# Liupeter01/Software-Rasterizer

Hardware: AMD Instinct MI355X
Metric: frames_per_sec (higher is better)
Workload: dtype f32

## Files before the change

software-rasterizer_amd/csrc/srz_api.hip:

```cpp
#include <dlfcn.h>

#include <algorithm>
#include <cmath>
#include <cstdio>
#include <cstdlib>
#include <cstring>
#include <initializer_list>
#include <new>
#include <string>
#include <vector>

#include "srz_device.h"

using namespace srz;

namespace {
std::string g_create_error;

struct EventPair {
  hipEvent_t t0, t1, t2, t3;
  bool detailed;
};

struct BatchDesc {
// ... 12 lines not shown

struct srz_ctx {
  int device = 0;
  hipStream_t stream = nullptr;
  std::string err;
  int shard_rank = 0, shard_world = 1;
  TexDesc h_tex[MAX_TEX];
  uint32_t *d_texmem[MAX_TEX];
  unsigned long long *d_stats = nullptr;
  struct MeshSlot {
    srz_vertex *d_verts = nullptr;
    uint32_t *d_faces = nullptr;
    uint32_t *d_corner_off = nullptr;
    uint32_t n_verts = 0, n_faces = 0;
    uint64_t upload = 0;
  } mesh[MAX_MESH];
  uint64_t mesh_uploads = 0;
  int timing = 0;
  std::vector<EventPair> ev_pool, ev_used;
  double acc_ms[4] = {0, 0, 0, 0};
  uint64_t tex_version = 1;
  int acc_launches = 0;
  std::vector<float> acc_samples;
  hipEvent_t span_t0 = nullptr;
  bool span_open = false;
  double span_ms = 0.0;
  unsigned long long dbg[ST_COUNT] = {};
  srz_frameset *draw_fs = nullptr;
  float *draw_out = nullptr;
  std::vector<uint64_t> draw_sig;
  int env_sub_batch = 0;
  bool env_no_packed = false;
  uint32_t env_clear_wgs = 0;
  std::vector<std::pair<uint64_t, uint32_t>> clear_memo;
  bool opt_approx_shade = false;
  bool opt_pool_lazy = false;
  static constexpr int EV_RING = 8;
  hipStream_t stream2 = nullptr;
  hipEvent_t ev_fork[EV_RING] = {}, ev_join[EV_RING] = {};
  float *batch_out = nullptr;
  size_t batch_out_bytes = 0;
  hipStream_t stream3 = nullptr;
  hipEvent_t ev_piece[EV_RING] = {};
  unsigned ev_next = 0;
  hipEvent_t ev_raster[EV_RING] = {};
  unsigned raster_next = 0;
  hipStream_t raster_last_stream = nullptr;
  bool raster_valid = false;
};

struct srz_target {
  int width = 0, height = 0;
  float *d_planes = nullptr;
  uint8_t *d_bgr8 = nullptr;
// ... 53 lines not shown
  std::vector<uint64_t> h_draw_upload;
  uint32_t n_draws = 0, max_faces = 0;
  uint64_t sdesc_version = 0;
  uint32_t tiles_x = 0, max_tiles = 0;
  bool have_stats = false;
  bool update_failed = false;
  static constexpr int CLEAR_TUNE_SKIP = 6, CLEAR_TUNE_AGAIN = 4096;
  struct ClearTune {
    uint32_t wgs = CLEAR_GRID_DEFAULT;
    bool done = false;
    int renders = 0;
    int since = 0;
    ClearCtl *d_ctl = nullptr;
    uint32_t *h_wgs = nullptr;
  } clear_tune;
  srz_stats stats{};
};

namespace {

hipStream_t pick_stream(const srz_ctx *ctx, void *stream) {
  if (!stream) return ctx->stream;
  return stream == SRZ_STREAM_NULL ? (hipStream_t) nullptr : (hipStream_t)stream;
}

int fail(srz_ctx *ctx, int code, const std::string &msg) {
  if (ctx)
    ctx->err = msg;
  else
    g_create_error = msg;
// ... 69 lines not shown
  for (int i = 0; i < srz_frameset::STAGE_RING; ++i) {
    if (fs->h_stage[i]) (void)hipHostFree(fs->h_stage[i]);
    if (fs->stage_ev[i]) (void)hipEventDestroy(fs->stage_ev[i]);
  }
  (void)hipFree(fs->d_dyn);
  (void)hipFree(fs->d_tris);
  (void)hipFree(fs->d_tri_pos);
  (void)hipFree(fs->d_bbox);
  (void)hipFree(fs->d_tri_batch);
  (void)hipFree(fs->d_pool);
  (void)hipFree(fs->d_pool_heads);
  if (fs->h_pool_heads) (void)hipHostFree(fs->h_pool_heads);
  if (fs->clear_tune.h_wgs) (void)hipHostFree(fs->clear_tune.h_wgs), fs->clear_tune.h_wgs = nullptr;
  if (fs->clear_tune.d_ctl) (void)hipFree(fs->clear_tune.d_ctl), fs->clear_tune.d_ctl = nullptr;
  (void)hipFree(fs->d_tile_info);
  (void)hipFree(fs->d_sparse_rows);
  (void)hipFree(fs->d_slow_list);
  (void)hipFree(fs->d_slow_count);
  (void)hipFree(fs->d_redo_list);
  (void)hipFree(fs->d_vis);
  (void)hipFree(fs->d_worklist);
  (void)hipFree(fs->d_work_count);
  (void)hipFree(fs->d_chunk_rows);
  (void)hipFree(fs->d_band_desc);
  (void)hipFree(fs->d_band_ent);
  (void)hipFree(fs->d_sdesc);
}

struct Pass {
  enum Kind { COLOUR, VISIBILITY, COUNTING, SIZE_ONLY, PEEL } kind = COLOUR;
// ... 217 lines not shown
  return SRZ_OK;
}

void end_clear_plan(srz_frameset *fs, const ClearPlan &p, hipStream_t s) {
  if (p.count) ++fs->clear_tune.renders;
  if (p.stamp) launch_clear_tune(fs->clear_tune.d_ctl, fs->clear_tune.h_wgs, s);
  if (p.rebase) launch_clear_rebase(fs->clear_tune.d_ctl, s);
}

struct RenderPlan {
  Pass pass;
  hipStream_t s;
  bool side, turns, vertex_setup;
  ClearPlan clear;
  EventPair *ep;
};

int enqueue_sub_batch(srz_ctx *ctx, srz_frameset *fs, const RenderPlan &r, RenderArgs &a, int f0, int n, int part) {
  const bool stats = r.pass.kind == Pass::COUNTING;
  const hipStream_t s = r.s;
  const size_t tpf = (size_t)fs->n_local_bands * fs->tiles_x;
  RenderArgs v = a;
  if (n != fs->n_frames) {
    const int fa = r.pass.f_begin + f0;
    v.frames += fa, v.n_frames = (uint32_t)n;
    v.vis += (size_t)fa * tpf * ((size_t)TILE * TILE);
    v.tile_info += (size_t)fa * tpf;
    v.out += (size_t)fa * a.frame_stride;
    v.work_cap = (uint32_t)((size_t)(n < 8 ? n : (n + 7) / 8) * tpf);
  }
  const uint32_t tiles = (uint32_t)((size_t)n * tpf);
  if (r.vertex_setup) launch_chunks(v, n, fs->max_tris, s);
  else launch_setup(v, n, fs->max_tris, stats, s);
  launch_bin(v, n, fs->max_tris, s);
  if (!fs->pool_sized && !stats) {
    HIP_TRY(ctx, copy_demand(fs, part, s));
    HIP_TRY(ctx, hipStreamSynchronize(s));
    const uint32_t need = max_pool_demand(fs, part, part + 1);
    if (need > fs->pool_sub_cap) {
      if (int rc = grow_pool(ctx, fs, need, 8u)) return rc;
      a.pool = v.pool = fs->d_pool, a.pool_sub_cap = v.pool_sub_cap = fs->pool_sub_cap;
      HIP_TRY(ctx, hipMemsetAsync(fs->d_pool_heads, 0, sizeof(uint32_t) * CNT_STRIDE * fs->pool_n_sub, s));
      launch_bin(v, n, fs->max_tris, s);
    }
  }
  if (r.pass.kind == Pass::SIZE_ONLY) return SRZ_OK;
  if (r.ep) HIP_TRY(ctx, hipEventRecord(r.ep->t1, s));
  const unsigned ev = r.side ? ctx->ev_next++ % srz_ctx::EV_RING : 0u;
  if (r.side) {
    HIP_TRY(ctx, hipEventRecord(ctx->ev_fork[ev], s));
    HIP_TRY(ctx, hipStreamWaitEvent(ctx->stream2, ctx->ev_fork[ev], 0));
    launch_clear(v, tiles, ctx->stream2, r.clear.wgs);
    HIP_TRY(ctx, copy_demand(fs, part, ctx->stream2));
    HIP_TRY(ctx, hipEventRecord(ctx->ev_join[ev], ctx->stream2));
  }
  if (r.pass.kind == Pass::PEEL) launch_peel(v, r.pass.d_prev + (v.out - a.out), n, s);
  else launch_raster(v, n, stats, s);
  if (r.turns) {
    HIP_TRY(ctx, hipEventRecord(ctx->ev_raster[ctx->raster_next++ % srz_ctx::EV_RING], s));
    ctx->raster_last_stream = s, ctx->raster_valid = true;
  }
  if (r.ep) HIP_TRY(ctx, hipEventRecord(r.ep->t2, s));
  if (r.pass.writes_visibility()) launch_visibility(v, tiles, s);
  else launch_shade(v, tiles, stats, fs->fast_kinds, fs->any_generic, fs->approx_shade, s);
  if (r.side) HIP_TRY(ctx, hipStreamWaitEvent(s, ctx->ev_join[ev], 0));
  else if (r.pass.kind == Pass::PEEL || !raster_four_waves(v))
    HIP_TRY(ctx, copy_demand(fs, part, s));
// ... 23 lines not shown
    if (int rc = begin_timing(ctx, ep, detailed, s)) return rc;
  if (stats) HIP_TRY(ctx, hipMemsetAsync(ctx->d_stats, 0, ST_COUNT * sizeof(unsigned long long), s));
  if (fs->max_tris == 0) {
    HIP_TRY(ctx, hipMemsetAsync(fs->d_work_count, 0, sizeof(uint32_t) * CNT_STRIDE * N_WORK_LISTS, s));
    HIP_TRY(ctx, hipMemsetAsync(fs->d_pool_heads, 0, sizeof(uint32_t) * CNT_STRIDE * fs->pool_n_sub, s));
    HIP_TRY(ctx, hipMemsetAsync(fs->d_slow_count, 0, 2 * sizeof(uint32_t), s));
  }
  const bool turns = !stats && !size_only && fs->max_tiles >= 8192;
  if (turns && !ctx->ev_raster[0])
    if (int rc = create_side(ctx, "render: raster events", nullptr, false, ctx->ev_raster)) return rc;
  if (turns && ctx->raster_valid && ctx->raster_last_stream != s) {
    HIP_TRY(ctx, hipStreamWaitEvent(s, ctx->ev_raster[(ctx->raster_next + srz_ctx::EV_RING - 1) % srz_ctx::EV_RING], 0));
    a.other_streams = 1u;
  }
  const bool vertex_setup = fs->d_draws != nullptr && !stats;
  if (fs->d_draws) launch_vertex(fs->d_draws, fs->n_draws, fs->max_faces, fs->d_tris, fs->d_tri_pos, fs->d_frames, vertex_setup ? fs->d_bbox : nullptr, s);
  const bool any_fused = any_frame_has(fs, flags_or, SRZ_FUSED_CLEAR), side = any_fused && fs->max_tiles >= 8192 && !size_only;
  if (side && !ctx->stream2)
    if (int rc = create_side(ctx, "render: clear stream", &ctx->stream2, true, ctx->ev_fork, ctx->ev_join)) return rc;
  if (!side && any_fused) a.clear_in_raster = 1u;
  RenderPlan r{pass, s, side, turns, vertex_setup, ClearPlan{}, detailed ? &ep : nullptr};
  if (side)
    if (int rc = plan_clear(ctx, fs, pass, detailed, s, r.clear)) return rc;
  a.clear_wgs_dev = r.clear.dev_wgs;
  const int n_all = pass.f_count < 0 ? fs->n_frames : pass.f_count;
  const int chunk = sub_batch_frames(ctx, fs, n_all, stats || detailed);
  for (int f0 = 0, part = 0; f0 < n_all; f0 += chunk, ++part)
    if (int rc = enqueue_sub_batch(ctx, fs, r, a, f0, std::min(chunk, n_all - f0), part)) return rc;
  if (!stats) fs->pool_sized = true;
  end_clear_plan(fs, r.clear, s);
  if (timed) {
    HIP_TRY(ctx, hipEventRecord(ep.t3, s));
    ctx->ev_used.push_back(ep);
  }
  HIP_TRY(ctx, hipGetLastError());
  return SRZ_OK;
}

int render_entry(const char *name, srz_ctx *ctx, srz_frameset *fs, void *d_out, size_t out_bytes, uint32_t flags, void *stream, Pass pass) {
  if (!ctx) return SRZ_E_INVALID;
  const std::string fn(name);
  if (!fs || !d_out) return fail(ctx, SRZ_E_INVALID, fn + ": null frameset / output");
  if (out_bytes < srz_frameset_out_bytes(ctx, fs)) return fail(ctx, SRZ_E_INVALID, fn + ": output buffer too small");
  if (((uintptr_t)d_out & 15u) != 0) return fail(ctx, SRZ_E_INVALID, fn + ": output must be 16-byte aligned");
// ... 322 lines not shown

void srz_destroy(srz_ctx *ctx) {
  if (!ctx) return;
  (void)hipSetDevice(ctx->device);
  (void)hipStreamSynchronize(ctx->stream);
  if (ctx->draw_fs) srz_frameset_destroy(ctx, ctx->draw_fs);
  (void)hipFree(ctx->draw_out);
  (void)hipFree(ctx->batch_out);
  if (ctx->span_t0) (void)hipEventDestroy(ctx->span_t0);
  for (auto &ep : ctx->ev_used) ctx->ev_pool.push_back(ep);
  for (auto &ep : ctx->ev_pool) (void)hipEventDestroy(ep.t0), (void)hipEventDestroy(ep.t1), (void)hipEventDestroy(ep.t2), (void)hipEventDestroy(ep.t3);
  for (int i = 0; i < MAX_TEX; ++i) (void)hipFree(ctx->d_texmem[i]);
  for (int i = 0; i < MAX_MESH; ++i) (void)hipFree(ctx->mesh[i].d_verts), (void)hipFree(ctx->mesh[i].d_faces), (void)hipFree(ctx->mesh[i].d_corner_off);
  (void)hipFree(ctx->d_stats);
  destroy_side(ctx->stream2, ctx->ev_fork, ctx->ev_join);
  destroy_side(ctx->stream3, ctx->ev_piece);
  destroy_side(nullptr, ctx->ev_raster);
  (void)hipStreamDestroy(ctx->stream);
  delete ctx;
}

const char *srz_last_error(const srz_ctx *ctx) { return ctx ? ctx->err.c_str() : g_create_error.c_str(); }

int srz_set_option(srz_ctx *ctx, int option, int value) {
  if (!ctx) return SRZ_E_INVALID;
  if (option == SRZ_OPT_POOL_LAZY)
    ctx->opt_pool_lazy = value != 0;
  else if (option == SRZ_OPT_APPROX_SHADE)
    ctx->opt_approx_shade = value != 0;
  else
// ... 187 lines not shown
    const uint64_t n_wgs = (uint64_t)((n_frames + 7) / 8 * 8) * fs->n_local_bands;
    uint32_t n_sub = 1;
    while (n_sub < 64u && (uint64_t)n_sub * 256u <= n_wgs) n_sub *= 2u;
    fs->pool_n_sub = n_sub;
    const uint64_t cap = std::min<uint64_t>((4ull * tri_off + 4096u) / n_sub + 64u, 0xfffffff0ull / n_sub);
    fs->pool_sub_cap = (uint32_t)cap;
    FS_TRY(dev_alloc((void **)&fs->d_pool, sizeof(uint32_t) * cap * n_sub));
    FS_TRY(dev_alloc((void **)&fs->d_pool_heads, sizeof(uint32_t) * CNT_STRIDE * 64));
    FS_TRY(hipHostMalloc((void **)&fs->h_pool_heads, sizeof(uint32_t) * CNT_STRIDE * 64 * srz_frameset::DEMAND_PARTS, hipHostMallocMapped | hipHostMallocCoherent));
    if (e == hipSuccess) std::memset(fs->h_pool_heads, 0, sizeof(uint32_t) * CNT_STRIDE * 64 * srz_frameset::DEMAND_PARTS);
    FS_TRY(dev_alloc((void **)&fs->clear_tune.d_ctl, sizeof(ClearCtl)));
    if (e == hipSuccess) FS_TRY(hipMemset(fs->clear_tune.d_ctl, 0, sizeof(ClearCtl)));
    FS_TRY(hipHostMalloc((void **)&fs->clear_tune.h_wgs, 64, hipHostMallocMapped | hipHostMallocCoherent));
    if (e == hipSuccess) *fs->clear_tune.h_wgs = 0u;
    FS_TRY(dev_alloc((void **)&fs->d_tile_info, sizeof(uint2) * fs->max_tiles));
    FS_TRY(dev_alloc((void **)&fs->d_slow_list, sizeof(uint32_t) * fs->max_tiles));
    FS_TRY(dev_alloc((void **)&fs->d_slow_count, 2 * sizeof(uint32_t)));
    FS_TRY(dev_alloc((void **)&fs->d_redo_list, sizeof(uint4) * fs->max_tiles));
  }
  FS_TRY(dev_alloc((void **)&fs->d_vis, sizeof(uint32_t) * (size_t)fs->max_tiles * ((size_t)TILE * TILE)));
  FS_TRY(ensure_worklists(fs));
  FS_TRY(dev_alloc((void **)&fs->d_work_count, sizeof(uint32_t) * CNT_STRIDE * N_WORK_LISTS));
  FS_TRY(dev_alloc((void **)&fs->d_sdesc, sizeof(ShadeDescG) * fs->h_batches.size()));
  std::vector<uint8_t> h_dyn(fs->dyn_bytes);
  stage_dyn(fs, h_dyn.data());
  FS_TRY(hipMemcpy(fs->d_dyn, h_dyn.data(), fs->dyn_bytes, hipMemcpyHostToDevice));
  if (tri_off) {
    if (copy_tris) FS_TRY(hipMemcpy(fs->d_tris, h_tris.data(), sizeof(srz_tri) * tri_off, hipMemcpyHostToDevice));
    if (!h_pos.empty()) FS_TRY(hipMemcpy(fs->d_tri_pos, h_pos.data(), sizeof(float) * h_pos.size(), hipMemcpyHostToDevice));
    FS_TRY(hipMemcpy(fs->d_tri_batch, h_tb.data(), sizeof(uint16_t) * tri_off, hipMemcpyHostToDevice));
// ... 39 lines not shown
  {
    std::vector<uint32_t> at(off, off + n_verts);
    for (uint32_t i = 0; i < 3u * n_faces; ++i) corners[at[faces[i]]++] = i;
  }
  srz_ctx::MeshSlot m;
  HIP_TRY(ctx, hipMalloc(&m.d_verts, sizeof(srz_vertex) * n_verts));
  hipError_t e = hipMalloc(&m.d_faces, sizeof(uint32_t) * 3 * (n_faces ? n_faces : 1));
  if (e == hipSuccess) e = hipMalloc(&m.d_corner_off, sizeof(uint32_t) * lists.size());
  if (e == hipSuccess) e = hipMemcpy(m.d_verts, verts, sizeof(srz_vertex) * n_verts, hipMemcpyHostToDevice);
  if (e == hipSuccess && n_faces) e = hipMemcpy(m.d_faces, faces, sizeof(uint32_t) * 3 * n_faces, hipMemcpyHostToDevice);
  if (e == hipSuccess) e = hipMemcpy(m.d_corner_off, lists.data(), sizeof(uint32_t) * lists.size(), hipMemcpyHostToDevice);
  if (e != hipSuccess) {
    (void)hipFree(m.d_verts), (void)hipFree(m.d_faces), (void)hipFree(m.d_corner_off);
    return fail(ctx, SRZ_E_NOMEM, std::string("srz_mesh_upload: ") + hipGetErrorString(e));
  }
  m.n_verts = n_verts, m.n_faces = n_faces, m.upload = ++ctx->mesh_uploads;
  (void)hipStreamSynchronize(ctx->stream);
  (void)hipFree(ctx->mesh[mesh_id].d_verts), (void)hipFree(ctx->mesh[mesh_id].d_faces), (void)hipFree(ctx->mesh[mesh_id].d_corner_off);
  ctx->mesh[mesh_id] = m;
  return SRZ_OK;
}

int srz_mesh_update(srz_ctx *ctx, int mesh_id, const srz_vertex *d_verts, uint32_t n_verts, void *stream) {
  if (!ctx) return SRZ_E_INVALID;
  const std::string fn("srz_mesh_update");
  if (mesh_id < 0 || mesh_id >= MAX_MESH || !ctx->mesh[mesh_id].d_verts) return fail(ctx, SRZ_E_INVALID, fn + ": no mesh in that slot");
  if (!d_verts) return fail(ctx, SRZ_E_INVALID, fn + ": null vertices");
  const srz_ctx::MeshSlot &m = ctx->mesh[mesh_id];
  if (n_verts != m.n_verts) return fail(ctx, SRZ_E_INVALID, fn + ": n_verts is not the slot's vertex count");
  if (!aligned<4>({d_verts})) return fail(ctx, SRZ_E_INVALID, fn + ": the vertices must be 4-byte aligned");
  HIP_TRY(ctx, hipSetDevice(ctx->device));
  HIP_TRY(ctx, hipMemcpyAsync(m.d_verts, d_verts, sizeof(srz_vertex) * n_verts, hipMemcpyDeviceToDevice, pick_stream(ctx, stream)));
  return SRZ_OK;
}

static int check_mesh_normals(srz_ctx *ctx, const std::string &fn, int mesh_id, const float *d_pos, uint32_t pos_stride, uint32_t n_sets,
                              MeshNormalsArgs &a, size_t *pos_span) {
  if (mesh_id < 0 || mesh_id >= MAX_MESH || !ctx->mesh[mesh_id].d_verts) return fail(ctx, SRZ_E_INVALID, fn + ": no mesh in that slot");
  const srz_ctx::MeshSlot &m = ctx->mesh[mesh_id];
  if (n_sets == 0u || n_sets > 65535u) return fail(ctx, SRZ_E_INVALID, fn + ": n_sets must be 1 .. 65535");
  if (!d_pos && n_sets != 1u) return fail(ctx, SRZ_E_INVALID, fn + ": the slot's own vertices are one set (n_sets must be 1)");
  if (d_pos && pos_stride < 3u) return fail(ctx, SRZ_E_INVALID, fn + ": pos_stride must be at least 3");
  a.pos = d_pos ? d_pos : reinterpret_cast<const float *>(m.d_verts), a.pos_stride = d_pos ? pos_stride : 8u;
  a.faces = m.d_faces, a.corner_off = m.d_corner_off, a.corners = m.d_corner_off + m.n_verts + 1;
  a.n_verts = m.n_verts, a.n_sets = n_sets;
  *pos_span = (((size_t)n_sets * m.n_verts - 1u) * a.pos_stride + 3u) * sizeof(float);
// ... 140 lines not shown
      const srz_ctx::MeshSlot &m = ctx->mesh[dr.mesh_id];
      DrawDesc dd{};
      dd.verts = m.d_verts, dd.faces = m.d_faces, dd.n_faces = m.n_faces, dd.tri_off = first, dd.frame = (uint32_t)f;
      set_draw(dd, sf, dr);
      draws.push_back(dd), draw_mesh.push_back(dr.mesh_id), draw_upload.push_back(m.upload);
      first += m.n_faces;
    }
  }
  std::vector<srz_frame> fr;
  std::vector<srz_batch> batches;
  scene_frames(ctx, frames, n_frames, fr, batches);
  srz_frameset *fs = nullptr;
  int rc = build_frameset(ctx, fr.data(), n_frames, &fs, false, false, &draws);
  if (rc) return rc;
  fs->h_draw_mesh = draw_mesh, fs->h_draw_upload = draw_upload;
  *out = fs;
  return size_pool ? size_pool_at_create(ctx, out) : SRZ_OK;
}

int srz_sceneset_update(srz_ctx *ctx, srz_frameset *fs, const srz_scene_frame *frames, int n_frames) {
  if (!ctx) return SRZ_E_INVALID;
  if (!fs || !frames || !fs->d_draws) return fail(ctx, SRZ_E_INVALID, "srz_sceneset_update: not a sceneset");
  if (n_frames != fs->n_frames) return fail(ctx, SRZ_E_INVALID, "srz_sceneset_update: frame count changed");
  HIP_TRY(ctx, hipSetDevice(ctx->device));
  for (int f = 0, di = 0; f < n_frames; ++f) {
    const srz_scene_frame &sf = frames[f];
    const FrameDesc &d = fs->h_frames[f];
    if (sf.width != fs->width || sf.height != fs->height || sf.n_lights != d.n_lights || sf.n_draws != d.n_batches ||
        (sf.n_lights && !sf.lights) || (sf.n_draws && !sf.draws))
      return fail(ctx, SRZ_E_INVALID, "srz_sceneset_update: structure changed");
    for (uint32_t k = 0; k < sf.n_draws; ++k, ++di) {
      const srz_mesh_draw &dr = sf.draws[k];
      if (dr.mesh_id != fs->h_draw_mesh[di] || dr.mesh_id < 0 || dr.mesh_id >= MAX_MESH ||
          ctx->mesh[dr.mesh_id].n_faces != fs->h_draws[di].n_faces || ctx->mesh[dr.mesh_id].upload != fs->h_draw_upload[di])
        return fail(ctx, SRZ_E_INVALID, "srz_sceneset_update: mesh binding changed");
    }
  }
  for (int f = 0, di = 0; f < n_frames; ++f)
    for (uint32_t k = 0; k < frames[f].n_draws; ++k) set_draw(fs->h_draws[di++], frames[f], frames[f].draws[k]);
  std::vector<srz_frame> fr;
  std::vector<srz_batch> batches;
  scene_frames(ctx, frames, n_frames, fr, batches);
  return refresh_frames(ctx, fs, fr.data(), n_frames, "srz_sceneset_update", false);
}

int srz_target_create(srz_ctx *ctx, int width, int height, srz_target **out) {
  if (!ctx) return SRZ_E_INVALID;
  if (!out || width <= 0 || height <= 0 || width > 32767 || height > 32767) return fail(ctx, SRZ_E_INVALID, "srz_target_create: bad size");
  *out = nullptr;
  HIP_TRY(ctx, hipSetDevice(ctx->device));
  srz_target *t = new (std::nothrow) srz_target();
  if (!t) return fail(ctx, SRZ_E_NOMEM, "srz_target_create: out of host memory");
  t->width = width, t->height = height;
  const size_t plane = (size_t)width * height;
// ... 1598 lines not shown
  unsigned long long h[5];
  HIP_TRY(ctx, hipMemcpyAsync(h, ctx->d_stats, sizeof h, hipMemcpyDeviceToHost, ctx->stream));
  HIP_TRY(ctx, hipStreamSynchronize(ctx->stream));
  for (int i = 0; i < 5; ++i) out5[i] = h[i];
  return SRZ_OK;
}

int srz_debug_counters(srz_ctx *ctx, uint64_t *out, int n) {
  if (!ctx || !out) return SRZ_E_INVALID;
#ifdef SRZ_PHASE_PROBE
  (void)hipDeviceSynchronize();
  (void)hipMemcpy(ctx->dbg, ctx->d_stats, sizeof ctx->dbg, hipMemcpyDeviceToHost);
  (void)hipMemset(ctx->d_stats, 0, sizeof ctx->dbg);
#endif
  for (int i = 0; i < n && i < ST_COUNT; ++i) out[i] = ctx->dbg[i];
  return ST_COUNT;
}

}
namespace {
struct RcclApi {
  void *handle = nullptr;
  struct UniqueId { char internal[128]; };
  int (*GetUniqueId)(UniqueId *) = nullptr;
  int (*CommInitRank)(void **, int, UniqueId, int) = nullptr;
  int (*AllGather)(const void *, void *, size_t, int, void *, hipStream_t) = nullptr;
  int (*CommDestroy)(void *) = nullptr;
  const char *(*GetErrorString)(int) = nullptr;
  std::string error;
};
RcclApi &rccl() {
// ... 305 lines not shown
  for (int f = 0; f < n_frames; ++f) {
    const srz_frame &fr = frames[f];
    const FrameDesc &d = fs->h_frames[f];
    if (fr.width != fs->width || fr.height != fs->height) return bad(SRZ_E_INVALID, "frame size changed");
    if (fr.n_lights != d.n_lights || (fr.n_lights && !fr.lights)) return bad(SRZ_E_INVALID, "light count changed");
    if (fr.n_batches != d.n_batches || (fr.n_batches && !fr.batches)) return bad(SRZ_E_INVALID, "batch count changed");
    for (uint32_t b = 0; b < fr.n_batches; ++b) {
      const srz_batch &sb = fr.batches[b];
      if (sb.n_tris != fs->h_batches[d.batch_off + b].count) return bad(SRZ_E_INVALID, "triangle count of a batch changed");
      if (sb.shader < SRZ_SHADER_NORMAL || sb.shader > SRZ_SHADER_BUMP) return bad(SRZ_E_INVALID, "unknown shader type");
      if (copy_tris && sb.n_tris && !sb.tris) return bad(SRZ_E_INVALID, "batch with null triangle pointer");
    }
  }
  if (int rc = ensure_stage_ring(ctx, fs, who)) return rc;
  bool batches_changed = false;
  for (int f = 0; f < n_frames; ++f) {
    const srz_frame &fr = frames[f];
    FrameDesc &d = fs->h_frames[f];
    set_shading(d, fr);
    if (fr.n_lights) std::memcpy(&fs->h_lights[d.light_off], fr.lights, sizeof(srz_light) * fr.n_lights);
    for (uint32_t b = 0; b < fr.n_batches; ++b) {
      BatchDesc &bd = fs->h_batches[d.batch_off + b];
      if (bd.shader != fr.batches[b].shader || bd.tex_id != fr.batches[b].tex_id)
        bd.shader = fr.batches[b].shader, bd.tex_id = fr.batches[b].tex_id, batches_changed = true;
    }
  }
  classify_frames(fs);
  fs->update_failed = ensure_worklists(fs) != hipSuccess;
  if (fs->update_failed) return bad(SRZ_E_NOMEM, "hipMalloc of the work lists failed");
  if (int rc = upload_dyn(ctx, fs)) return rc;
  if (batches_changed) fs->sdesc_version = 0;
  if (copy_tris) {
    for (int f = 0; f < n_frames; ++f) {
      size_t o = fs->h_frames[f].tri_off;
      for (uint32_t b = 0; b < frames[f].n_batches; ++b) {
        const srz_batch &sb = frames[f].batches[b];
        if (sb.n_tris) HIP_TRY(ctx, hipMemcpyAsync(fs->d_tris + o, sb.tris, sizeof(srz_tri) * sb.n_tris, hipMemcpyHostToDevice, ctx->stream));
        o += sb.n_tris;
      }
    }
  }
// ... 146 lines not shown
```

software-rasterizer_amd/csrc/srz_device.h:

```cpp
#pragma once
#include <hip/hip_runtime.h>
#include <stdint.h>

#include "../../include/srz.h"

namespace srz {

constexpr int TILE = 32;
constexpr int BAND = 32;
constexpr int KEY_STRIDE = TILE + 1;
constexpr int LDS_STRIDE = 32;
#ifndef SRZ_BAND_ROT
#define SRZ_BAND_ROT 5
#endif
__host__ __device__ inline int band_rot(int world) { return (SRZ_BAND_ROT % world) ? SRZ_BAND_ROT : (SRZ_BAND_ROT ? 1 : 0); }
__host__ __device__ inline int band_of(int lb, int rank, int world) {
  if (world == 1) return lb;
  int j = (rank - band_rot(world) * lb) % world;
  return lb * world + (j < 0 ? j + world : j);
}
__host__ __device__ inline int rank_of_band(int b, int world) { return (b + band_rot(world) * (b / world)) % world; }
constexpr uint32_t NO_TRI = 0xffffffffu;
constexpr uint32_t CNT_STRIDE = 32;
constexpr uint32_t FD_FAST_SHADE = 0x100u, FD_NL_SHIFT = 9;
// ... 89 lines not shown
  uint4 *redo_list;
  uint32_t *redo_count;
  uint32_t *vis;
  uint4 *worklist;
  uint64_t kind_slots;
  uint32_t *work_count;
  uint32_t work_cap;
  uint32_t tiles_x, n_local_bands, n_frames;
  float *out;
  uint64_t frame_stride;
  uint32_t local_rows;
  int32_t shard_rank, shard_world;
  uint32_t flags_or;
  unsigned long long *stats;
  const uint32_t *clear_wgs_dev;
};

constexpr int CLEAR_CANDS = 3, CLEAR_TUNE_BLOCK = 3, CLEAR_TUNE_RENDERS = 2 * CLEAR_CANDS * CLEAR_TUNE_BLOCK;
constexpr uint32_t CLEAR_CAND[CLEAR_CANDS] = {96, 128, 256};
constexpr uint32_t CLEAR_GRID_MAX = 256, CLEAR_GRID_DEFAULT = 96;
struct ClearCtl {
  uint32_t wgs;
  uint32_t cur, pos, phase, done, alive;
  uint32_t n[CLEAR_CANDS];
  unsigned long long last;
  float t[CLEAR_CANDS][4];
  float score[CLEAR_CANDS];
};
void launch_clear_tune(ClearCtl *ctl, uint32_t *h_wgs, hipStream_t s);
void launch_clear_rebase(ClearCtl *ctl, hipStream_t s);

// ... 50 lines not shown
  const float *attr;
  float *out;
  const float *gout;
  float *gattr;
  uint64_t attr_frame_stride;
  uint32_t n_verts, n_ch, pos_tris, n_frames;
};
void launch_corner_attr(const CornerAttrArgs &a, hipStream_t s);
void launch_corner_attr_grad(const CornerAttrArgs &a, hipStream_t s);
void launch_chunks(const RenderArgs &a, int n_frames, uint32_t max_tris, hipStream_t s);
void launch_setup(const RenderArgs &a, int n_frames, uint32_t max_tris, bool stats, hipStream_t s);
void launch_bin(const RenderArgs &a, int n_frames, uint32_t max_tris, hipStream_t s);
void launch_raster(const RenderArgs &a, int n_frames, bool stats, hipStream_t s);
void launch_peel(const RenderArgs &a, const float *prev, int n_frames, hipStream_t s);
bool raster_four_waves(const RenderArgs &a);
void launch_clear(const RenderArgs &a, uint32_t max_tiles, hipStream_t s, uint32_t wgs);
void launch_shade(const RenderArgs &a, uint32_t max_tiles, bool stats, uint32_t kinds, bool any_generic, bool approx, hipStream_t s);
void launch_visibility(const RenderArgs &a, uint32_t max_tiles, hipStream_t s);
struct ShadeVisArgs {
  const FrameDesc *frames;
  const srz_tri *tris;
  const uint16_t *tri_batch;
  const srz_light *lights;
  const ShadeDescG *sdesc;
  const float *vis;
  float *out;
  uint64_t frame_stride;
  uint32_t local_rows, tiles_x, n_local_bands, n_frames;
  int32_t shard_rank, shard_world;
  uint32_t flags_or, in_place;
  uint32_t any_generic;
// ... 439 lines not shown
```

software-rasterizer_amd/csrc/srz_kernels.hip:

```cpp
#include "srz_device.h"

#include <algorithm>
#include <cstdio>
#include <cstdlib>
#include <type_traits>

#pragma clang fp contract(off)

namespace srz {

#define SRZ_CAS __attribute__((address_space(4)))
template <typename T> __device__ __forceinline__ const SRZ_CAS T *as_const(const T *p) { return (const SRZ_CAS T *)(p); }
typedef float f32x4 __attribute__((ext_vector_type(4)));
typedef unsigned int u32x2 __attribute__((ext_vector_type(2)));
typedef unsigned int u32x4 __attribute__((ext_vector_type(4)));

__device__ __forceinline__ float sse_max(float a, float b) { return a > b ? a : b; }
__device__ __forceinline__ float sse_min(float a, float b) { return a < b ? a : b; }
__device__ __forceinline__ float std_max(float a, float b) { return (a < b) ? b : a; }
__device__ __forceinline__ float std_clamp(float v, float lo, float hi) { return (v < lo) ? lo : (hi < v) ? hi : v; }
__device__ __forceinline__ float fmsubf(float a, float b, float c) { return __builtin_fmaf(a, b, -c); }
__device__ __forceinline__ float fmaf_(float a, float b, float c) { return __builtin_fmaf(a, b, c); }

__device__ __forceinline__ uint32_t f2u_(float f) { return __builtin_bit_cast(uint32_t, f); }
// ... 2215 lines not shown
    float *gz = rc.out0 + (size_t)ly * W + x4;
    const bool full = vec_ok && x4 + 3 <= rc.tx1;
    if (tile_has_owner)
      quad_store(gz, rc.plane, {z4}, full, x4, rc.tx1);
    else
      quad_store(gz, rc.plane, {z4, zero4, zero4, zero4}, full, x4, rc.tx1);
  }
  if (tile_has_owner) {
    uint32_t *slot = a.vis + ((size_t)frame * tiles_per_frame + tile) * PIX_SLOT;
    for (int it = 0; it < 4; ++it) ids_store4(slot, (uint32_t)((it * 8 + (lane >> 3)) * TILE + (lane & 7) * 4), id4[it], false, false);
    if (lane == 0) work_append(a, fd->flags, frame * tiles_per_frame + tile, work_entry(frame, lb, tx, false, false, 0u, 0u));
  }
}

__global__ __launch_bounds__(256) void k_clear(RenderArgs a) {
  const uint32_t n_items = a.n_frames * a.n_local_bands * 4u;
  const float inf = __builtin_inff();
  uint32_t n_wgs = gridDim.x;
  if (a.clear_wgs_dev) {
    const uint32_t w = *as_const(a.clear_wgs_dev);
    n_wgs = min(w ? w : CLEAR_CAND[0], gridDim.x);
    if (blockIdx.x >= n_wgs) return;
  }
  for (uint32_t it = blockIdx.x; it < n_items; it += n_wgs) {
    const uint32_t br = it >> 2, pl = it & 3u;
    const uint32_t f = br / a.n_local_bands, lb = br % a.n_local_bands;
    const SRZ_CAS FrameDesc *fd = as_const(a.frames) + f;
    if (!((fd->flags | a.flags_or) & SRZ_FUSED_CLEAR)) continue;
    const int W = fd->width, H = fd->height;
    const int band = band_of((int)lb, a.shard_rank, a.shard_world);
    const int rows = min(BAND, H - band * BAND);
    const size_t plane = (size_t)a.local_rows * (size_t)W;
    float *base = a.out + (size_t)f * a.frame_stride + (size_t)lb * BAND * (size_t)W + pl * plane;
    const float v = pl == 0u ? inf : 0.f;
    const float4 v4 = make_float4(v, v, v, v);
    const SRZ_CAS u32x2 *cnt = as_const(reinterpret_cast<const u32x2 *>(a.tile_info)) + (size_t)br * a.tiles_x;
    for (int x4 = (int)threadIdx.x * 4; x4 < W; x4 += (int)blockDim.x * 4) {
      if (cnt[(uint32_t)x4 / TILE].x != 0u) continue;
      if (((W & 3) == 0)) {
        for (int ly = 0; ly < rows; ++ly) store_nt(base + (size_t)ly * W + x4, v4);
      } else {
        for (int ly = 0; ly < rows; ++ly)
          for (int k = 0; k < 4 && x4 + k < W; ++k) base[(size_t)ly * W + x4 + k] = v;
      }
    }
  }
}


#ifndef SRZ_FAST_MINW
#define SRZ_FAST_MINW 6
#endif
#ifndef SRZ_STAGE_TRIS
// ... 5332 lines not shown
  }
  int arg = -1;
  for (int i = 0; i < CLEAR_CANDS; ++i)
    if ((c->alive >> i & 1u) && (arg < 0 || c->score[i] < c->score[arg])) arg = i;
  c->wgs = CLEAR_CAND[arg < 0 ? 0 : arg], c->done = 1u;
  __hip_atomic_store(h_wgs, c->wgs, __ATOMIC_RELEASE, __HIP_MEMORY_SCOPE_SYSTEM);
}

void launch_clear_tune(ClearCtl *ctl, uint32_t *h_wgs, hipStream_t s) { hipLaunchKernelGGL(k_clear_tune, dim3(1), dim3(1), 0, s, ctl, h_wgs); }

__global__ void k_clear_rebase(ClearCtl *c) {
  if (!c->done) c->last = __builtin_amdgcn_s_memrealtime();
}
void launch_clear_rebase(ClearCtl *ctl, hipStream_t s) { hipLaunchKernelGGL(k_clear_rebase, dim3(1), dim3(1), 0, s, ctl); }

void launch_clear(const RenderArgs &a, uint32_t max_tiles, hipStream_t s, uint32_t wgs) {
  if (max_tiles == 0) return;
  const uint32_t n_items = a.n_frames * a.n_local_bands * 4u;
  const uint32_t cap = wgs ? wgs : 96u;
  hipLaunchKernelGGL(k_clear, dim3(n_items < cap ? n_items : cap), dim3(256), 0, s, a);
}

static uint32_t tile_grid(uint32_t items, uint32_t cap = 16384u) { return (std::min(items, cap) + 7u) & ~7u; }

static dim3 shade_grid(const RenderArgs &a, uint32_t max_tiles) { return dim3(tile_grid(max_tiles, a.other_streams ? 2048u : 16384u)); }

template <int FASTNL, bool BUMPY, class L> static void launch_kind(uint32_t kinds, bool approx, L &launch) {
  if (!((kinds >> build_kind<FASTNL, BUMPY>()) & 1u)) return;
  if constexpr (FASTNL > 0 && !BUMPY)
    if (approx) return launch(std::integral_constant<int, FASTNL>{}, std::false_type{}, std::true_type{});
  launch(std::integral_constant<int, FASTNL>{}, std::bool_constant<BUMPY>{}, std::false_type{});
}
template <class L> static void launch_fast_kinds(uint32_t kinds, bool approx, L &&launch) {
  launch_kind<1, false>(kinds, approx, launch), launch_kind<2, false>(kinds, approx, launch);
  launch_kind<3, false>(kinds, approx, launch), launch_kind<4, false>(kinds, approx, launch);
// ... 177 lines not shown
```

Before: 331,600.

## Start fused clear early using cached per-tile coverage mask across renders

Adds a per-frame, per-band bitmask of tiles that have triangles. It is rebuilt only when geometry, the eye position or the meshes change. When the mask is valid, the first slice of the clear kernel is launched on the side stream before vertex setup and binning, and the rest after binning, so clearing overlaps geometry work instead of waiting behind it. Vertex launch is moved into the sub-batch path. The risk is a stale mask if a geometry change is missed, which would produce wrong output, plus the cost of extra events and a mask-build kernel.

```diff
diff --git a/software-rasterizer_amd/csrc/srz_api.hip b/software-rasterizer_amd/csrc/srz_api.hip
--- a/software-rasterizer_amd/csrc/srz_api.hip
+++ b/software-rasterizer_amd/csrc/srz_api.hip
@@ -50,8 +50,11 @@
     uint32_t *d_corner_off = nullptr;
     uint32_t n_verts = 0, n_faces = 0;
     uint64_t upload = 0;
+    uint64_t moved = 0;
   } mesh[MAX_MESH];
   uint64_t mesh_uploads = 0;
+  uint64_t mesh_moves = 0;
+  unsigned long long early_clears = 0, mask_refreshes = 0;
   int timing = 0;
   std::vector<EventPair> ev_pool, ev_used;
   double acc_ms[4] = {0, 0, 0, 0};
@@ -74,6 +77,7 @@
   static constexpr int EV_RING = 8;
   hipStream_t stream2 = nullptr;
   hipEvent_t ev_fork[EV_RING] = {}, ev_join[EV_RING] = {};
+  hipEvent_t ev_bin[EV_RING] = {};
   float *batch_out = nullptr;
   size_t batch_out_bytes = 0;
   hipStream_t stream3 = nullptr;
@@ -157,6 +161,10 @@
     ClearCtl *d_ctl = nullptr;
     uint32_t *h_wgs = nullptr;
   } clear_tune;
+  uint32_t *d_clear_mask = nullptr;
+  uint32_t mask_words = 0;
+  uint64_t geom_gen = 1, mask_gen = 0, mask_moves = 0;
+  std::vector<int> h_mesh_slots;
   srz_stats stats{};
 };
 
@@ -256,6 +264,7 @@
   if (fs->clear_tune.h_wgs) (void)hipHostFree(fs->clear_tune.h_wgs), fs->clear_tune.h_wgs = nullptr;
   if (fs->clear_tune.d_ctl) (void)hipFree(fs->clear_tune.d_ctl), fs->clear_tune.d_ctl = nullptr;
   (void)hipFree(fs->d_tile_info);
+  (void)hipFree(fs->d_clear_mask);
   (void)hipFree(fs->d_sparse_rows);
   (void)hipFree(fs->d_slow_list);
   (void)hipFree(fs->d_slow_count);
@@ -503,7 +512,14 @@
   bool side, turns, vertex_setup;
   ClearPlan clear;
   EventPair *ep;
+  bool early = false;
+  bool refresh_mask = false;
 };
+
+bool clear_mask_valid(const srz_ctx *ctx, const srz_frameset *fs) {
+  if (!fs->d_clear_mask || fs->mask_gen != fs->geom_gen) return false;
+  return std::none_of(fs->h_mesh_slots.begin(), fs->h_mesh_slots.end(), [&](int m) { return ctx->mesh[m].moved > fs->mask_moves; });
+}
 
 int enqueue_sub_batch(srz_ctx *ctx, srz_frameset *fs, const RenderPlan &r, RenderArgs &a, int f0, int n, int part) {
   const bool stats = r.pass.kind == Pass::COUNTING;
@@ -519,6 +535,20 @@
     v.work_cap = (uint32_t)((size_t)(n < 8 ? n : (n + 7) / 8) * tpf);
   }
   const uint32_t tiles = (uint32_t)((size_t)n * tpf);
+  uint32_t *const mask = fs->d_clear_mask ? fs->d_clear_mask + (size_t)(r.pass.f_begin + f0) * fs->n_local_bands * fs->mask_words : nullptr;
+  v.mask_words = fs->mask_words;
+  const uint32_t front_of = fs->d_draws ? CLEAR_FRONT_OF / 2u : CLEAR_FRONT_OF;
+  const unsigned ev = r.side ? ctx->ev_next++ % srz_ctx::EV_RING : 0u;
+  if (r.early) {
+    HIP_TRY(ctx, hipEventRecord(ctx->ev_fork[ev], s));
+    HIP_TRY(ctx, hipStreamWaitEvent(ctx->stream2, ctx->ev_fork[ev], 0));
+    RenderArgs c = v;
+    c.clear_mask = mask;
+    launch_clear(c, tiles, ctx->stream2, r.clear.wgs, 0, 1, front_of);
+    ++ctx->early_clears;
+  }
+  if (f0 == 0 && fs->d_draws)
+    launch_vertex(fs->d_draws, fs->n_draws, fs->max_faces, fs->d_tris, fs->d_tri_pos, fs->d_frames, r.vertex_setup ? fs->d_bbox : nullptr, s);
   if (r.vertex_setup) launch_chunks(v, n, fs->max_tris, s);
   else launch_setup(v, n, fs->max_tris, stats, s);
   launch_bin(v, n, fs->max_tris, s);
@@ -533,13 +563,18 @@
       launch_bin(v, n, fs->max_tris, s);
     }
   }
+  if (r.refresh_mask) launch_clear_mask(v, mask, s);
   if (r.pass.kind == Pass::SIZE_ONLY) return SRZ_OK;
   if (r.ep) HIP_TRY(ctx, hipEventRecord(r.ep->t1, s));
-  const unsigned ev = r.side ? ctx->ev_next++ % srz_ctx::EV_RING : 0u;
   if (r.side) {
-    HIP_TRY(ctx, hipEventRecord(ctx->ev_fork[ev], s));
-    HIP_TRY(ctx, hipStreamWaitEvent(ctx->stream2, ctx->ev_fork[ev], 0));
-    launch_clear(v, tiles, ctx->stream2, r.clear.wgs);
+    hipEvent_t *const behind_bin = r.early ? ctx->ev_bin : ctx->ev_fork;
+    HIP_TRY(ctx, hipEventRecord(behind_bin[ev], s));
+    HIP_TRY(ctx, hipStreamWaitEvent(ctx->stream2, behind_bin[ev], 0));
+    if (r.early) {
+      RenderArgs c = v;
+      c.clear_mask = mask;
+      launch_clear(c, tiles, ctx->stream2, r.clear.wgs, 1, front_of, front_of);
+    } else launch_clear(v, tiles, ctx->stream2, r.clear.wgs);
     HIP_TRY(ctx, copy_demand(fs, part, ctx->stream2));
     HIP_TRY(ctx, hipEventRecord(ctx->ev_join[ev], ctx->stream2));
   }
@@ -593,7 +628,6 @@
     a.other_streams = 1u;
   }
   const bool vertex_setup = fs->d_draws != nullptr && !stats;
-  if (fs->d_draws) launch_vertex(fs->d_draws, fs->n_draws, fs->max_faces, fs->d_tris, fs->d_tri_pos, fs->d_frames, vertex_setup ? fs->d_bbox : nullptr, s);
   const bool any_fused = any_frame_has(fs, flags_or, SRZ_FUSED_CLEAR), side = any_fused && fs->max_tiles >= 8192 && !size_only;
   if (side && !ctx->stream2)
     if (int rc = create_side(ctx, "render: clear stream", &ctx->stream2, true, ctx->ev_fork, ctx->ev_join)) return rc;
@@ -602,11 +636,17 @@
   if (side)
     if (int rc = plan_clear(ctx, fs, pass, detailed, s, r.clear)) return rc;
   a.clear_wgs_dev = r.clear.dev_wgs;
+  const bool mask_valid = clear_mask_valid(ctx, fs);
+  r.early = side && mask_valid && !a.other_streams;
+  r.refresh_mask = fs->d_clear_mask && !mask_valid && !stats && pass.f_count < 0;
+  if (r.early && !ctx->ev_bin[0])
+    if (int rc = create_side(ctx, "render: clear events", nullptr, false, ctx->ev_bin)) return rc;
   const int n_all = pass.f_count < 0 ? fs->n_frames : pass.f_count;
   const int chunk = sub_batch_frames(ctx, fs, n_all, stats || detailed);
   for (int f0 = 0, part = 0; f0 < n_all; f0 += chunk, ++part)
     if (int rc = enqueue_sub_batch(ctx, fs, r, a, f0, std::min(chunk, n_all - f0), part)) return rc;
   if (!stats) fs->pool_sized = true;
+  if (r.refresh_mask) fs->mask_gen = fs->geom_gen, fs->mask_moves = ctx->mesh_moves, ++ctx->mask_refreshes;
   end_clear_plan(fs, r.clear, s);
   if (timed) {
     HIP_TRY(ctx, hipEventRecord(ep.t3, s));
@@ -959,6 +999,7 @@
   for (int i = 0; i < MAX_MESH; ++i) (void)hipFree(ctx->mesh[i].d_verts), (void)hipFree(ctx->mesh[i].d_faces), (void)hipFree(ctx->mesh[i].d_corner_off);
   (void)hipFree(ctx->d_stats);
   destroy_side(ctx->stream2, ctx->ev_fork, ctx->ev_join);
+  destroy_side(nullptr, ctx->ev_bin);
   destroy_side(ctx->stream3, ctx->ev_piece);
   destroy_side(nullptr, ctx->ev_raster);
   (void)hipStreamDestroy(ctx->stream);
@@ -1176,6 +1217,8 @@
     FS_TRY(hipHostMalloc((void **)&fs->clear_tune.h_wgs, 64, hipHostMallocMapped | hipHostMallocCoherent));
     if (e == hipSuccess) *fs->clear_tune.h_wgs = 0u;
     FS_TRY(dev_alloc((void **)&fs->d_tile_info, sizeof(uint2) * fs->max_tiles));
+    fs->mask_words = (fs->tiles_x + 31u) / 32u;
+    if (fs->max_tiles >= 8192) FS_TRY(dev_alloc((void **)&fs->d_clear_mask, sizeof(uint32_t) * (size_t)n_frames * fs->n_local_bands * fs->mask_words));
     FS_TRY(dev_alloc((void **)&fs->d_slow_list, sizeof(uint32_t) * fs->max_tiles));
     FS_TRY(dev_alloc((void **)&fs->d_slow_count, 2 * sizeof(uint32_t)));
     FS_TRY(dev_alloc((void **)&fs->d_redo_list, sizeof(uint4) * fs->max_tiles));
@@ -1245,7 +1288,7 @@
     (void)hipFree(m.d_verts), (void)hipFree(m.d_faces), (void)hipFree(m.d_corner_off);
     return fail(ctx, SRZ_E_NOMEM, std::string("srz_mesh_upload: ") + hipGetErrorString(e));
   }
-  m.n_verts = n_verts, m.n_faces = n_faces, m.upload = ++ctx->mesh_uploads;
+  m.n_verts = n_verts, m.n_faces = n_faces, m.upload = ++ctx->mesh_uploads, m.moved = ++ctx->mesh_moves;
   (void)hipStreamSynchronize(ctx->stream);
   (void)hipFree(ctx->mesh[mesh_id].d_verts), (void)hipFree(ctx->mesh[mesh_id].d_faces), (void)hipFree(ctx->mesh[mesh_id].d_corner_off);
   ctx->mesh[mesh_id] = m;
@@ -1261,6 +1304,7 @@
   if (n_verts != m.n_verts) return fail(ctx, SRZ_E_INVALID, fn + ": n_verts is not the slot's vertex count");
   if (!aligned<4>({d_verts})) return fail(ctx, SRZ_E_INVALID, fn + ": the vertices must be 4-byte aligned");
   HIP_TRY(ctx, hipSetDevice(ctx->device));
+  ctx->mesh[mesh_id].moved = ++ctx->mesh_moves;
   HIP_TRY(ctx, hipMemcpyAsync(m.d_verts, d_verts, sizeof(srz_vertex) * n_verts, hipMemcpyDeviceToDevice, pick_stream(ctx, stream)));
   return SRZ_OK;
 }
@@ -1431,6 +1475,8 @@
   int rc = build_frameset(ctx, fr.data(), n_frames, &fs, false, false, &draws);
   if (rc) return rc;
   fs->h_draw_mesh = draw_mesh, fs->h_draw_upload = draw_upload;
+  std::sort(draw_mesh.begin(), draw_mesh.end());
+  fs->h_mesh_slots.assign(draw_mesh.begin(), std::unique(draw_mesh.begin(), draw_mesh.end()));
   *out = fs;
   return size_pool ? size_pool_at_create(ctx, out) : SRZ_OK;
 }
@@ -1455,6 +1501,7 @@
   }
   for (int f = 0, di = 0; f < n_frames; ++f)
     for (uint32_t k = 0; k < frames[f].n_draws; ++k) set_draw(fs->h_draws[di++], frames[f], frames[f].draws[k]);
+  ++fs->geom_gen;
   std::vector<srz_frame> fr;
   std::vector<srz_batch> batches;
   scene_frames(ctx, frames, n_frames, fr, batches);
@@ -3083,7 +3130,9 @@
   (void)hipMemset(ctx->d_stats, 0, sizeof ctx->dbg);
 #endif
   for (int i = 0; i < n && i < ST_COUNT; ++i) out[i] = ctx->dbg[i];
-  return ST_COUNT;
+  if (n > ST_COUNT) out[ST_COUNT] = ctx->early_clears;
+  if (n > ST_COUNT + 1) out[ST_COUNT + 1] = ctx->mask_refreshes;
+  return ST_COUNT + 2;
 }
 
 }
@@ -3419,9 +3468,11 @@
   }
   if (int rc = ensure_stage_ring(ctx, fs, who)) return rc;
   bool batches_changed = false;
+  bool geom_changed = copy_tris;
   for (int f = 0; f < n_frames; ++f) {
     const srz_frame &fr = frames[f];
     FrameDesc &d = fs->h_frames[f];
+    geom_changed = geom_changed || std::memcmp(d.eye, fr.eye, sizeof d.eye) != 0;
     set_shading(d, fr);
     if (fr.n_lights) std::memcpy(&fs->h_lights[d.light_off], fr.lights, sizeof(srz_light) * fr.n_lights);
     for (uint32_t b = 0; b < fr.n_batches; ++b) {
@@ -3430,6 +3481,7 @@
         bd.shader = fr.batches[b].shader, bd.tex_id = fr.batches[b].tex_id, batches_changed = true;
     }
   }
+  if (geom_changed) ++fs->geom_gen;
   classify_frames(fs);
   fs->update_failed = ensure_worklists(fs) != hipSuccess;
   if (fs->update_failed) return bad(SRZ_E_NOMEM, "hipMalloc of the work lists failed");
diff --git a/software-rasterizer_amd/csrc/srz_device.h b/software-rasterizer_amd/csrc/srz_device.h
--- a/software-rasterizer_amd/csrc/srz_device.h
+++ b/software-rasterizer_amd/csrc/srz_device.h
@@ -127,7 +127,11 @@
   uint32_t flags_or;
   unsigned long long *stats;
   const uint32_t *clear_wgs_dev;
-};
+  const uint32_t *clear_mask;
+  uint32_t mask_words;
+  uint32_t clear_it0, clear_it1;
+};
+void launch_clear_mask(const RenderArgs &a, uint32_t *mask, hipStream_t s);
 
 constexpr int CLEAR_CANDS = 3, CLEAR_TUNE_BLOCK = 3, CLEAR_TUNE_RENDERS = 2 * CLEAR_CANDS * CLEAR_TUNE_BLOCK;
 constexpr uint32_t CLEAR_CAND[CLEAR_CANDS] = {96, 128, 256};
@@ -208,7 +212,12 @@
 void launch_raster(const RenderArgs &a, int n_frames, bool stats, hipStream_t s);
 void launch_peel(const RenderArgs &a, const float *prev, int n_frames, hipStream_t s);
 bool raster_four_waves(const RenderArgs &a);
-void launch_clear(const RenderArgs &a, uint32_t max_tiles, hipStream_t s, uint32_t wgs);
+#ifndef SRZ_CLEAR_FRONT_OF
+#define SRZ_CLEAR_FRONT_OF 16
+#endif
+constexpr uint32_t CLEAR_FRONT_OF = SRZ_CLEAR_FRONT_OF;
+static_assert(CLEAR_FRONT_OF >= 4u && CLEAR_FRONT_OF % 2u == 0u, "SRZ_CLEAR_FRONT_OF: a sceneset's front is twice a frameset's");
+void launch_clear(const RenderArgs &a, uint32_t max_tiles, hipStream_t s, uint32_t wgs, uint32_t it0_of = 0, uint32_t it1_of = 1, uint32_t of = 1);
 void launch_shade(const RenderArgs &a, uint32_t max_tiles, bool stats, uint32_t kinds, bool any_generic, bool approx, hipStream_t s);
 void launch_visibility(const RenderArgs &a, uint32_t max_tiles, hipStream_t s);
 struct ShadeVisArgs {
diff --git a/software-rasterizer_amd/csrc/srz_kernels.hip b/software-rasterizer_amd/csrc/srz_kernels.hip
--- a/software-rasterizer_amd/csrc/srz_kernels.hip
+++ b/software-rasterizer_amd/csrc/srz_kernels.hip
@@ -2253,7 +2253,7 @@
 }
 
 __global__ __launch_bounds__(256) void k_clear(RenderArgs a) {
-  const uint32_t n_items = a.n_frames * a.n_local_bands * 4u;
+  const uint32_t n_items = a.clear_it1;
   const float inf = __builtin_inff();
   uint32_t n_wgs = gridDim.x;
   if (a.clear_wgs_dev) {
@@ -2261,7 +2261,7 @@
     n_wgs = min(w ? w : CLEAR_CAND[0], gridDim.x);
     if (blockIdx.x >= n_wgs) return;
   }
-  for (uint32_t it = blockIdx.x; it < n_items; it += n_wgs) {
+  for (uint32_t it = a.clear_it0 + blockIdx.x; it < n_items; it += n_wgs) {
     const uint32_t br = it >> 2, pl = it & 3u;
     const uint32_t f = br / a.n_local_bands, lb = br % a.n_local_bands;
     const SRZ_CAS FrameDesc *fd = as_const(a.frames) + f;
@@ -2274,8 +2274,11 @@
     const float v = pl == 0u ? inf : 0.f;
     const float4 v4 = make_float4(v, v, v, v);
     const SRZ_CAS u32x2 *cnt = as_const(reinterpret_cast<const u32x2 *>(a.tile_info)) + (size_t)br * a.tiles_x;
+    const SRZ_CAS uint32_t *mask = a.clear_mask ? as_const(a.clear_mask) + (size_t)br * a.mask_words : nullptr;
     for (int x4 = (int)threadIdx.x * 4; x4 < W; x4 += (int)blockDim.x * 4) {
-      if (cnt[(uint32_t)x4 / TILE].x != 0u) continue;
+      if (mask) {
+        if ((mask[(uint32_t)x4 / (TILE * 32u)] >> ((uint32_t)x4 / TILE & 31u)) & 1u) continue;
+      } else if (cnt[(uint32_t)x4 / TILE].x != 0u) continue;
       if (((W & 3) == 0)) {
         for (int ly = 0; ly < rows; ++ly) store_nt(base + (size_t)ly * W + x4, v4);
       } else {
@@ -7638,11 +7641,30 @@
 }
 void launch_clear_rebase(ClearCtl *ctl, hipStream_t s) { hipLaunchKernelGGL(k_clear_rebase, dim3(1), dim3(1), 0, s, ctl); }
 
-void launch_clear(const RenderArgs &a, uint32_t max_tiles, hipStream_t s, uint32_t wgs) {
+void launch_clear(const RenderArgs &a, uint32_t max_tiles, hipStream_t s, uint32_t wgs, uint32_t it0_of, uint32_t it1_of, uint32_t of) {
   if (max_tiles == 0) return;
   const uint32_t n_items = a.n_frames * a.n_local_bands * 4u;
   const uint32_t cap = wgs ? wgs : 96u;
-  hipLaunchKernelGGL(k_clear, dim3(n_items < cap ? n_items : cap), dim3(256), 0, s, a);
+  auto cut = [&](uint32_t k) { return k >= of ? n_items : (uint32_t)((uint64_t)n_items * k / of) & ~7u; };
+  RenderArgs c = a;
+  c.clear_it0 = cut(it0_of), c.clear_it1 = cut(it1_of);
+  if (c.clear_it0 >= c.clear_it1) return;
+  const uint32_t n = c.clear_it1 - c.clear_it0;
+  hipLaunchKernelGGL(k_clear, dim3(n < cap ? n : cap), dim3(256), 0, s, c);
+}
+
+__global__ __launch_bounds__(256) void k_clear_mask(RenderArgs a, uint32_t *mask) {
+  const uint32_t i = blockIdx.x * 256u + threadIdx.x;
+  if (i >= a.n_frames * a.n_local_bands * a.mask_words) return;
+  const uint32_t br = i / a.mask_words, tx0 = i % a.mask_words * 32u;
+  const SRZ_CAS u32x2 *cnt = as_const(reinterpret_cast<const u32x2 *>(a.tile_info)) + (size_t)br * a.tiles_x;
+  uint32_t bits = 0;
+  for (uint32_t b = 0; b < 32u && tx0 + b < a.tiles_x; ++b) bits |= (cnt[tx0 + b].x != 0u ? 1u : 0u) << b;
+  mask[i] = bits;
+}
+void launch_clear_mask(const RenderArgs &a, uint32_t *mask, hipStream_t s) {
+  const uint32_t n = a.n_frames * a.n_local_bands * a.mask_words;
+  if (n) hipLaunchKernelGGL(k_clear_mask, dim3((n + 255u) / 256u), dim3(256), 0, s, a, mask);
 }
 
 static uint32_t tile_grid(uint32_t items, uint32_t cap = 16384u) { return (std::min(items, cap) + 7u) & ~7u; }
```

Measured after the change: 332,800, median of 4. About the same (+0.4%).
